# krea-ai/realtime-video

Hardware: AMD Instinct MI355X
Metric: frames/sec at 832x480, 4-step 14B T2V (per-step DiT latency in config) (higher is better)
Workload: dtype bf16

## Files before the change

__graft_entry__.py:

```python
import os
import sys

ROOT = os.path.dirname(os.path.abspath(__file__))
if ROOT not in sys.path:
    sys.path.insert(0, ROOT)


def build() -> None:
    from realtime_video_amd import _lib
    _lib.build(verbose=False)
    import realtime_video_amd.attention
    import realtime_video_amd.causal_model
    import realtime_video_amd.pipeline
    import realtime_video_amd.session
    import realtime_video_amd.taehv
    import realtime_video_amd.vae_decoder
    lib = _lib.load()
    missing = [s for s in _lib.declared_symbols() if not hasattr(lib, s)]
    if missing:
        raise RuntimeError(f"librtv_hip.so lacks symbols declared in include/rtv_hip.h: {missing}")
    import re
    import subprocess
    def audit(script, *argv, **env):
        r = subprocess.run([os.path.join(ROOT, "scripts", "micro", script), *argv], capture_output=True, text=True,
                           env=dict(os.environ, **env))
        return r.stdout + ("\n[stderr]\n" + r.stderr if r.stderr.strip() else "") + (f"\n[exit {r.returncode}]" if r.returncode else "")

    out = audit("w4_audit.sh", "600", W4_AUDIT_DIR=os.path.join(ROOT, "realtime_video_amd", "csrc", "build", "w4_audit"))
    ok = all(re.search(pat, out) for pat in (r"accumulation register outside asm: 0\b", r"v_accvgpr outside asm: 0\b", r"\bscratch 0\b",
                                              r"vgpr_spill_count: 0\b", r"private_segment_fixed_size: 0\b"))
    if not ok:
        raise RuntimeError("attn_w4 audit failed (scripts/micro/w4_audit.sh):\n" + out)
    out = audit("g5_audit.sh", G5_AUDIT_DIR=os.path.join(ROOT, "realtime_video_amd", "csrc", "build", "g5_audit"))
    if len(re.findall(r"AUDIT gemm5 F16=\d: vgpr_spills 0 private_segment 0 scratch_ops 0 mfma 120 compiler_acc_refs_before_last_accumulator_read 0 ", out)) != 2:
        raise RuntimeError("gemm5 audit failed (scripts/micro/g5_audit.sh):\n" + out)
    out = audit("h4_audit.sh", H4_AUDIT_DIR=os.path.join(ROOT, "realtime_video_amd", "csrc", "build", "h4_audit"))
    if len(re.findall(r"AUDIT _ZN3rtv1[78]conv_halo4p?_kernel\S*: arch_vgprs \d+ vgpr_spills 0 sgpr_spills \d+ private_segment 0 scratch_ops 0 "
                      r"mfma 216 compiler_acc_refs 0 \(a0-a7: 0\)", out)) != 2:
        raise RuntimeError("conv_halo4 audit failed (scripts/micro/h4_audit.sh):\n" + out)
    print(f"build ok: {_lib.LIB_PATH} ({len(_lib.declared_symbols())} C-ABI symbols; attn_w4 / gemm5 / conv_halo4 register audits clean)")


def smoke() -> None:
    import torch
    from oracle import vae_oracle as vo
    from oracle import wan_oracle as wo
    from realtime_video_amd.causal_model import CausalWanModel
    from realtime_video_amd.vae_decoder import VAEDecoderWrapper
    from realtime_video_amd.wan_wrapper import WanDiffusionWrapper

    assert torch.cuda.is_available(), "smoke() needs a GPU"
    dev = "cuda:0"
    torch.cuda.set_device(0)
    cfg = dict(dim=256, ffn_dim=512, num_heads=2, num_layers=1, freq_dim=256, text_len=512, eps=1e-6)
    w = wo.make_weights(cfg, seed=1, text_dim=64)
    g = torch.Generator().manual_seed(2)
    lat = torch.randn(1, 3, 16, 60, 104, generator=g).to(torch.bfloat16)
    ctx = torch.randn(32, 64, generator=g).to(torch.bfloat16)
    t = torch.tensor([[500.0, 500.0, 500.0]])
    kvc = wo.initialize_kv_cache(1, 1, 9360, 2, 128, torch.bfloat16)
    cac = wo.initialize_crossattn_cache(1, 1, 2, 128, torch.bfloat16)
    ref, _ = wo.wrapper_forward(w, cfg, wo.FlowMatchScheduler(), lat, [ctx], t, kvc, cac, 0)

    model = CausalWanModel(dim=256, ffn_dim=512, num_heads=2, num_layers=1, text_dim=64, device=dev)
    model.load_state_dict(w)
    wr = WanDiffusionWrapper(model, timestep_shift=5.0)
    kv = [{"k": torch.zeros(1, 9360, 2, 128, dtype=torch.bfloat16, device=dev),
           "v": torch.zeros(1, 9360, 2, 128, dtype=torch.bfloat16, device=dev), "global_end_index": 0, "local_end_index": 0}]
    ca = [{"k": torch.zeros(1, 512, 2, 128, dtype=torch.bfloat16, device=dev),
           "v": torch.zeros(1, 512, 2, 128, dtype=torch.bfloat16, device=dev), "is_init": False}]
    flow, _ = wr(lat.to(dev), {"prompt_embeds": [ctx.to(dev)]}, t.to(dev), kv, ca, current_start=0)
    torch.cuda.synchronize()
    err = float((flow.cpu().double() - ref.double()).norm() / ref.double().norm())
# ... 20 lines not shown
```

realtime_video_amd/_lib.py:

```python
import ctypes
import os
import re
import subprocess

_HERE = os.path.dirname(os.path.abspath(__file__))
LIB_PATH = os.environ.get("RTV_LIB_PATH") or os.path.join(_HERE, "librtv_hip.so")
CSRC = os.path.join(_HERE, "csrc")

_INCLUDE = os.path.join(os.path.dirname(_HERE), "include")
HEADERS = ("rtv_hip.h", "rtv_hip_lab.h")

_lib = None

_SCALARS = {"int": ctypes.c_int, "int64_t": ctypes.c_int64, "float": ctypes.c_float, "double": ctypes.c_double,
            "size_t": ctypes.c_size_t}
_RETURNS = {"int": ctypes.c_int, "size_t": ctypes.c_size_t, "const char*": ctypes.c_char_p}
_STARS = r"(\*(?:\s*const\s*\*)?)?"


def _field_type(base, stars, structs):
    value = _SCALARS.get(base) or structs.get(base)
    if not stars:
        return value
    if base == "void":
# ... 57 lines not shown

STRUCTS, PROTOTYPES = {}, {}
for _name in HEADERS:
    PROTOTYPES.update(parse_header(_read(_name), STRUCTS))
IO_HEADER = "rtv_hip_io.h"
IO_STRUCTS = dict(STRUCTS)
IO_PROTOTYPES = parse_header(_read(IO_HEADER), IO_STRUCTS)
IO_STRUCTS = {k: v for k, v in IO_STRUCTS.items() if k not in STRUCTS}
JPEG_HEADER = "rtv_hip_jpeg.h"
JPEG_STRUCTS = dict(STRUCTS)
JPEG_PROTOTYPES = parse_header(_read(JPEG_HEADER), JPEG_STRUCTS)
JPEG_STRUCTS = {k: v for k, v in JPEG_STRUCTS.items() if k not in STRUCTS}
JPEGDEC_HEADER = "rtv_hip_jpeg_decode.h"
JPEGDEC_STRUCTS = dict(STRUCTS)
JPEGDEC_PROTOTYPES = parse_header(_read(JPEGDEC_HEADER), JPEGDEC_STRUCTS)
JPEGDEC_STRUCTS = {k: v for k, v in JPEGDEC_STRUCTS.items() if k not in STRUCTS}
LORA_HEADER = "rtv_hip_lora.h"
LORA_STRUCTS = dict(STRUCTS)
LORA_PROTOTYPES = parse_header(_read(LORA_HEADER), LORA_STRUCTS)
LORA_STRUCTS = {k: v for k, v in LORA_STRUCTS.items() if k not in STRUCTS}
CROSS_FOLD_HEADER = "rtv_hip_cross_fold.h"
CROSS_FOLD_STRUCTS = dict(STRUCTS)
CROSS_FOLD_PROTOTYPES = parse_header(_read(CROSS_FOLD_HEADER), CROSS_FOLD_STRUCTS)
FP8_ROWS_HEADER = "rtv_hip_fp8_rows.h"
FP8_ROWS_PROTOTYPES = parse_header(_read(FP8_ROWS_HEADER), dict(STRUCTS))
ATTN_FP8_HEADER = "rtv_hip_attn_fp8.h"
ATTN_FP8_STRUCTS = dict(STRUCTS)
ATTN_FP8_PROTOTYPES = parse_header(_read(ATTN_FP8_HEADER), ATTN_FP8_STRUCTS)
ATTN_FP8_STRUCTS = {k: v for k, v in ATTN_FP8_STRUCTS.items() if k not in STRUCTS}
MXFP4_HEADER = "rtv_hip_mxfp4.h"
MXFP4_PROTOTYPES = parse_header(_read(MXFP4_HEADER), dict(STRUCTS))
MXFP6_HEADER = "rtv_hip_mxfp6.h"
MXFP6_PROTOTYPES = parse_header(_read(MXFP6_HEADER), dict(STRUCTS))
LORA_MAX_ADAPTERS, LORA_MAX_RANK = (int(re.search(rf"^#define\s+RTV_LORA_MAX_{n}\s+(\d+)", _read(LORA_HEADER), flags=re.M).group(1))
                                    for n in ("ADAPTERS", "RANK"))
FRAMES_MAX = int(re.search(r"^#define\s+RTV_FRAMES_MAX\s+(\d+)", _read(IO_HEADER), flags=re.M).group(1))
ABI_VERSION = int(re.search(r"^#define\s+RTV_ABI_VERSION\s+(\d+)", _read(HEADERS[0]), flags=re.M).group(1))


def build(verbose=False):
    jobs = os.environ.get("MAX_JOBS") or str(min(16, len(os.sched_getaffinity(0)) if hasattr(os, "sched_getaffinity") else os.cpu_count() or 4))
    cmd = ["make", "-C", CSRC, "-j", jobs]
    res = subprocess.run(cmd, capture_output=True, text=True)
    if verbose or res.returncode != 0:
        print(res.stdout[-4000:])
        print(res.stderr[-4000:])
    if res.returncode != 0:
        raise RuntimeError("building librtv_hip.so failed")
    return LIB_PATH


def declared_symbols(lab=True):
    out = set()
    for name in HEADERS if lab else HEADERS[:1]:
        text = re.sub(r"/\*.*?\*/", "", _read(name), flags=re.S)
        out.update(re.findall(r"\b(rtv_[a-z0-9_]+)\s*\(", text))
    return sorted(out)


def load():
    global _lib
    if _lib is not None:
        return _lib
    if not os.path.exists(LIB_PATH):
        raise RuntimeError(
            f"{LIB_PATH} is missing: run `python -c 'import __graft_entry__ as g; g.build()'` "
            "(or `make -C realtime_video_amd/csrc`). There is no CPU fallback for the HIP path.")
    lib = ctypes.CDLL(LIB_PATH)
    for name, (restype, argtypes) in list(PROTOTYPES.items()) + list(IO_PROTOTYPES.items()) + list(JPEG_PROTOTYPES.items()) + list(JPEGDEC_PROTOTYPES.items()) + list(LORA_PROTOTYPES.items()) + list(CROSS_FOLD_PROTOTYPES.items()) + list(FP8_ROWS_PROTOTYPES.items()) + list(ATTN_FP8_PROTOTYPES.items()) + list(MXFP4_PROTOTYPES.items()) + list(MXFP6_PROTOTYPES.items()):
        fn = getattr(lib, name, None)
        if fn is None:
            if os.environ.get("RTV_LIB_PATH"):
                continue
            raise RuntimeError(f"librtv_hip.so does not export {name}")
        fn.restype, fn.argtypes = restype, argtypes
    have = lib.rtv_version()
    if have != ABI_VERSION:
        raise RuntimeError(f"{LIB_PATH} reports ABI revision {have}, include/rtv_hip.h declares RTV_ABI_VERSION {ABI_VERSION}: "
                           "rebuild the library (`make -C realtime_video_amd/csrc`)")
    _lib = lib
    return lib


def check(status, what):
    if status != 0:
        msg = load().rtv_last_error().decode("utf-8", "replace")
        raise RuntimeError(f"{what} failed (status {status}): {msg}")


def call(name, *args):
    check(getattr(load(), name)(*args), name)
```

realtime_video_amd/csrc/dit_forward.hip:

```cpp
#include <atomic>
#include <string>

#include "../../include/rtv_hip_attn_fp8.h"
#include "../../include/rtv_hip_mxfp4.h"
#include "../../include/rtv_hip_mxfp6.h"
#include "rtv_common.h"
#include "rtv_internal.h"

namespace rtv {

__global__ void silu_kernel(const bf16_t* __restrict__ x, bf16_t* __restrict__ out, int64_t n) {
  for (int64_t i = (int64_t)blockIdx.x * blockDim.x + threadIdx.x; i < n; i += (int64_t)gridDim.x * blockDim.x)
    out[i] = f32_to_bf16(silu(bf16_to_f32(x[i])));
}

constexpr int FOLD_ROWS = 64, FOLD_LD = 130;
__global__ __launch_bounds__(256) void cross_fold_weight_kernel(const bf16_t* __restrict__ w, int64_t ldw, const bf16_t* __restrict__ v,
                                                               int64_t ldv, bf16_t* __restrict__ vo, int64_t ldvo, int H, int rows, int kh,
                                                               int k_fold) {
  __shared__ __attribute__((aligned(16))) bf16_t sW[FOLD_ROWS * FOLD_LD];
  __shared__ __attribute__((aligned(16))) bf16_t sV[128 * FOLD_LD];
  const int tid = threadIdx.x, lane = tid & 63, wave = tid >> 6;
  const int n0 = blockIdx.x * FOLD_ROWS, h = blockIdx.y;
  for (int id = tid; id < FOLD_ROWS * 64; id += 256) {
// ... 290 lines not shown
  const int pk = cfg->in_dim * 4;
  RTV_TRY(rtv_patchify(st->x, b.prow, cfg->in_dim, F, c.gh, c.gw, stream));
  RTV_TRY(linear(c, -1, b.prow + (size_t)c.r0 * pk, pk, w->patch_w, w->patch_b, b.x, c.rc, d, 0, nullptr, 0, 0, 0, nullptr, tc, stream));
  RTV_TRY(rtv_sinusoidal_embedding(st->t, b.sinus, F, cfg->freq_dim, stream));
  RTV_TRY(linear(c, S_TIME0, b.sinus, cfg->freq_dim, w->time0_w, w->time0_b, b.te1, F, d, RTV_ACT_SILU, nullptr, 0, 0, 0, nullptr, tc, stream));
  RTV_TRY(linear(c, S_TIME2, b.te1, d, w->time2_w, w->time2_b, b.e, F, d, 0, nullptr, 0, 0, 0, nullptr, tc, stream));
  RTV_TRY(rtv_silu(b.e, b.se, (int64_t)F * d, stream));
  RTV_TRY(linear(c, S_TPROJ, b.se, d, w->tproj_w, w->tproj_b, b.e0, F, 6 * d, 0, nullptr, 0, 0, 0, nullptr, tc, stream));
  RTV_TRY(rtv_modulation_table(w->modulation, b.e0, b.emod, L, F, 6, 6, d, stream));
  RTV_TRY(rtv_modulation_table(w->head_modulation, b.e, b.ehead, 1, F, 2, 1, d, stream));
  if (st->compute_cross_kv) {
    if (!st->context) return set_error(-1, "dit: context required to initialise the cross-attention cache");
    const int T = cfg->text_len;
    RTV_TRY(linear(c, S_TEXT0, st->context, cfg->text_dim, w->text0_w, w->text0_b, b.ctx1, T, d, RTV_ACT_GELU_TANH, nullptr, 0, 0, 0, nullptr, tc, stream));
    RTV_TRY(linear(c, S_TEXT2, b.ctx1, d, w->text2_w, w->text2_b, b.ctx, T, d, 0, nullptr, 0, 0, 0, nullptr, tc, stream));
    for (int l = 0; l < L; ++l) {
      const rtv_dit_layer_weights& lw = w->layers[l];
      RTV_TRY(linear(c, S_LAYER0 + S_PER_LAYER * l + S_CK, b.ctx, d, lw.ck_w, lw.ck_b, b.ktmp, T, d, 0, nullptr, 0, 0, 0, nullptr, tc, stream));
      RTV_TRY(rtv_rmsnorm(b.ktmp, d, st->ca_k[l], d, T, d, cfg->eps, lw.cnorm_k_w, stream));
      RTV_TRY(linear(c, S_LAYER0 + S_PER_LAYER * l + S_CV, b.ctx, d, lw.cv_w, lw.cv_b, st->ca_v[l], T, d, 0, nullptr, 0, 0, 0, nullptr, tc, stream));
      if (c.fold_k)
        RTV_TRY(rtv_cross_fold_weight(lw.co_w, d, st->ca_v[l], d, st->ca_v[c.L + l], st->ca_vo_ld, c.H, st->text_rows + 1, c.fold_kh, c.fold_k,
                                      stream));
    }
  }
  return 0;
}

static int hp_check(Ctx& c, int world);
static int quantize_written_rows(Ctx& c, int l);

static std::atomic<void*> g_capture_q{nullptr}, g_capture_o{nullptr};
static std::atomic<int> g_direct_v{1};
static int dit_layer_proj(Ctx& c, int l, int parts, int world, void* q_send, void* kv_send) {
  const rtv_dit_layer_weights& lw = c.w->layers[l];
  const rtv_dit_step* st = c.st;
  DitBuffers& b = c.b;
  const int d = c.d;
  if (!(parts & (RTV_PROJ_LN | RTV_PROJ_Q | RTV_PROJ_KV))) return set_error(-1, "dit: empty projection phase");
  const uint16_t* em = b.emod + (size_t)l * c.F * 6 * d;
  if (parts & RTV_PROJ_LN) {
    const void* ln_out;
    RTV_TRY(ln_input(c, em + 0 * d, em + 1 * d, 6 * d, nullptr, nullptr, &ln_out));
  }
  const bool q = parts & RTV_PROJ_Q, kv = parts & RTV_PROJ_KV;
  if (!q && !kv) return 0;
  const int n0 = q ? 0 : d, nn = (q ? d : 0) + (kv ? 2 * d : 0);
  bool v_in_place = false;
  {
    void* v_dst = nullptr;
    if (kv && !kv_send && g_direct_v.load(std::memory_order_relaxed) && st->kv_v[l] && !(st->kv_row_stride & 7)) {
      int r0 = st->cache_row0 + c.r0;
      const int S = st->ring_lo, R = st->ring_size;
      bool one_range = true;
      if (R > 0 && r0 + c.rc > S) {
        if (r0 < S) one_range = false;
        else {
          r0 = S + (r0 - S + st->ring_shift) % R;
          one_range = r0 + c.rc <= S + R;
        }
      }
      uint16_t* dst = (uint16_t*)st->kv_v[l] + (size_t)r0 * st->kv_row_stride;
      if (one_range && !((uintptr_t)dst & 15)) v_dst = dst;
    }
    {
      const int rp = (q ? 1 : 0) | (kv ? 2 : 0) | (v_dst ? 4 : 0);
      if (q_send || kv_send) {
        RTV_TRY(hp_check(c, world));
        const int gc = d / world;
        if ((q && !q_send) || (kv && !kv_send)) return set_error(-1, "dit: exchange buffers required");
        RTV_TRY(qk_norm_rope_check(2 * gc, 0, c.rc, d, c.H, c.F, c.gh, c.gw, st->start_frame, c.r0, gc, (int64_t)c.rc * gc,
                                   (int64_t)c.rc * 2 * gc, 0, 0, 0, rp));
      } else {
        RTV_TRY(qk_norm_rope_check(st->kv_row_stride, st->cache_row0, c.rc, d, c.H, c.F, c.gh, c.gw, st->start_frame, c.r0, 0, 0, 0,
                                   st->ring_lo, st->ring_size, st->ring_shift, rp));
      }
    }
    const int sidx = S_LAYER0 + S_PER_LAYER * l + S_QKV;
    const void* a = c.cfg->use_fp8 >= FP8_ROWS ? nullptr : b.xn;
    RTV_TRY(quantize_input(c, sidx, a, c.rc, d, c.stream));
    auto proj = [&](int w_row0, int N, void* out, int ldc) {
      return project(c, sidx, a, d, lw.qkv_w, w_row0, lw.qkv_b, out, ldc, c.rc, N, 0, nullptr, 0, 0, 0, nullptr, c.tc, c.stream);
    };
    if (v_dst) {
      if (2 * d > n0) RTV_TRY(proj(n0, 2 * d - n0, b.qkv + n0, 3 * d));
      RTV_TRY(proj(2 * d, d, v_dst, (int)st->kv_row_stride));
      v_in_place = true;
    } else {
      RTV_TRY(proj(n0, nn, b.qkv + n0, 3 * d));
    }
  }
  const int rope_parts = (q ? 1 : 0) | (kv ? 2 : 0) | (v_in_place ? 4 : 0);
  if (q_send || kv_send) {
    RTV_TRY(hp_check(c, world));
    const int gc = d / world;
    if ((q && !q_send) || (kv && !kv_send)) return set_error(-1, "dit: exchange buffers required");
    return qk_norm_rope_launch(b.qkv, q_send, kv_send, kv_send ? (void*)((uint16_t*)kv_send + gc) : nullptr, 2 * gc, 0, c.rc, d, c.H,
                               c.cfg->eps, lw.norm_q_w, lw.norm_k_w, c.w->rope_cs, c.F, c.gh, c.gw, st->start_frame, c.r0, gc,
                               (int64_t)c.rc * gc, (int64_t)c.rc * 2 * gc, 0, 0, 0, rope_parts, c.stream);
  }
  RTV_TRY(qk_norm_rope_launch(b.qkv, b.q, st->kv_k[l], st->kv_v[l], st->kv_row_stride, st->cache_row0, c.rc, d, c.H, c.cfg->eps,
                              lw.norm_q_w, lw.norm_k_w, c.w->rope_cs, c.F, c.gh, c.gw, st->start_frame, c.r0, 0, 0, 0, st->ring_lo,
                              st->ring_size, st->ring_shift, rope_parts, c.stream));
  if (kv && c.fp8) return quantize_written_rows(c, l);
  return 0;
}

static int quantize_written_rows(Ctx& c, int l) {
  const rtv_dit_step* st = c.st;
  const rtv_attn_fp8_shadow* sh = c.fp8;
  if (!sh->k8[l] || !sh->v8t[l]) return set_error(-1, "dit: fp8 attention: a layer has no shadow");
  int a = st->cache_row0 + c.r0, n = c.rc;
  const int S = st->ring_lo, R = st->ring_size;
  int seg[3][2], ns = 0;
  if (R <= 0) {
    seg[ns][0] = a, seg[ns++][1] = n;
  } else {
    if (a < S) {
      const int m = n < S - a ? n : S - a;
      seg[ns][0] = a, seg[ns++][1] = m;
      a += m, n -= m;
    }
    if (n > 0) {
      const int p0 = S + (a - S + st->ring_shift) % R;
      const int first = n < S + R - p0 ? n : S + R - p0;
      seg[ns][0] = p0, seg[ns++][1] = first;
      if (n - first > R) return set_error(-1, "dit: fp8 attention: a call writes more rows than the ring holds");
      if (n > first) seg[ns][0] = S, seg[ns++][1] = n - first;
    }
  }
  void* amax = sh->amax ? sh->amax[l] : nullptr;
  for (int i = 0; i < ns; ++i)
    RTV_TRY(rtv_attn_quantize_kv(st->kv_k[l], st->kv_v[l], st->kv_row_stride, seg[i][0], seg[i][1], c.H, sh->k8[l], sh->v8t[l],
                                 sh->cache_rows, sh->k_scale, sh->v_scale, amax, c.stream));
  return 0;
}
// ... 236 lines not shown
  RTV_TRY(dit_begin(c));
  for (int l = 0; l < c.L; ++l) {
    if (st->kv_only && l == c.L - 1)
      return dit_layer_proj(c, l, RTV_PROJ_LN | RTV_PROJ_KV, 0, nullptr, nullptr);
    RTV_TRY(dit_layer_qkv(c, l));
    RTV_TRY(dit_layer_rest(c, l));
  }
  RTV_TRY(dit_head(c, c.b.hrow));
  return rtv_unpatchify(c.b.hrow, st->out, cfg->out_dim, c.F, c.gh, c.gw, stream);
}

extern "C" int rtv_dit_forward(const rtv_dit_config* cfg, const rtv_dit_weights* w, const rtv_dit_step* st,
                               void* workspace, size_t workspace_bytes, rtv_stream_t stream) {
  return dit_forward(cfg, w, st, nullptr, workspace, workspace_bytes, stream);
}

extern "C" int rtv_dit_forward_attn_fp8(const rtv_dit_config* cfg, const rtv_dit_weights* w, const rtv_dit_step* st,
                                        const rtv_attn_fp8_shadow* shadow, void* workspace, size_t workspace_bytes,
                                        rtv_stream_t stream) {
  if (!shadow) return set_error(-1, "dit: fp8 attention needs its shadow (rtv_attn_fp8_shadow)");
  return dit_forward(cfg, w, st, shadow, workspace, workspace_bytes, stream);
}

extern "C" int rtv_dit_lab_capture_self_attn(void* q_copy, void* o_copy) {
  g_capture_q = q_copy;
  g_capture_o = o_copy;
  return 0;
}

extern "C" int rtv_dit_set_direct_v(int on) {
  g_direct_v = on ? 1 : 0;
  return 0;
}
```

realtime_video_amd/csrc/elementwise.hip:

```cpp
#include "ln_row.h"
#include "rtv_common.h"
#include "rtv_internal.h"

namespace rtv {

static std::atomic<int> g_rope_wave{-1};
constexpr int ROPE_WAVE_MIN_ROWS = 2048;

__global__ __launch_bounds__(EW_THREADS) void layernorm_modulate_kernel(
    const bf16_t* __restrict__ x, bf16_t* __restrict__ out, int d, float eps,
    const bf16_t* __restrict__ shift, const bf16_t* __restrict__ scale, int frame_stride,
    int rows_per_frame, int row_offset, const bf16_t* __restrict__ weight, const bf16_t* __restrict__ bias) {
  __shared__ float red[8];
  bf16_t* orow = out + (size_t)blockIdx.x * d;
  layernorm_row(x, d, eps, shift, scale, frame_stride, rows_per_frame, row_offset, weight, bias, red,
                [&](int, int c, const float* o) { *(u32x4*)(orow + c * 8) = pack_bf16x8(o); });
}

__global__ __launch_bounds__(EW_THREADS) void rmsnorm_kernel(const bf16_t* __restrict__ x, int ldx,
                                                             bf16_t* __restrict__ out, int ldo, int d,
                                                             float eps,
                                                             const bf16_t* __restrict__ weight) {
  __shared__ float red[8];
  const int row = blockIdx.x;
// ... 35 lines not shown
}

constexpr int ROWS_PER_WG = 4;

struct RopeArgs {
  const bf16_t* qkv;
  bf16_t* q_out;
  bf16_t* k_cache;
  bf16_t* v_cache;
  int64_t cache_row_stride;
  int cache_row0;
  int M, d, hd;
  float eps;
  const bf16_t* wq;
  const bf16_t* wk;
  const float2* rope_cs;
  int gh, gw, start_frame, row_offset;
  int group_cols;
  int64_t q_group_stride, kv_group_stride;
  int ring_lo, ring_size, ring_shift;
  int parts;
};

__device__ __forceinline__ void rope8(float* x, const float2* w) {
#pragma unroll
  for (int t = 0; t < 4; ++t) {
    const float a = x[2 * t], b = x[2 * t + 1];
    x[2 * t] = a * w[t].x - b * w[t].y;
    x[2 * t + 1] = a * w[t].y + b * w[t].x;
  }
}

template <int CPL, bool LANE_CS>
__global__ __launch_bounds__(EW_THREADS) __attribute__((amdgpu_waves_per_eu(CPL <= 10 ? 5 : 3, 8))) void qk_norm_rope_cache_kernel(RopeArgs a) {
  const int lane = threadIdx.x & 63;
  const bool do_q = a.parts & 1, do_kv = a.parts & 2;
  const int nroles = do_kv ? 2 : 1;
  const int wid = __builtin_amdgcn_readfirstlane(blockIdx.x * ROWS_PER_WG + (threadIdx.x >> 6));
  const int row = wid / nroles, role = wid - row * nroles;
  if (row >= a.M) return;
  const int d = a.d;
  const int nchunks = d >> 3;
  const bf16_t* qr = a.qkv + (size_t)row * 3 * d;
  const bf16_t* vr = qr + 2 * d;
  const bool norm = role == 1 || do_q;
  const bf16_t* xr = role == 1 ? qr + d : qr;
  const bf16_t* wx = role == 1 ? a.wk : a.wq;

  const int half = a.hd >> 1;
  const int c1 = half / 3, c0 = half - 2 * c1;
  const int per_frame = a.gh * a.gw;
  const int grow = a.row_offset + row;
  const int f = grow / per_frame;
  const int rem = grow - f * per_frame;
  const int pos_h = rem / a.gw, pos_w = rem - pos_h * a.gw;
  const int pos_f = a.start_frame + f;
  auto load_cs = [&](int col, float2* w) {
    const int pj0 = (col % a.hd) >> 1;
#pragma unroll
    for (int t = 0; t < 4; ++t) {
      const int pj = pj0 + t;
      const int pos = pj < c0 ? pos_f : (pj < c0 + c1 ? pos_h : pos_w);
      w[t] = a.rope_cs[pos * half + pj];
    }
  };
  float2 cs[4];
  if (LANE_CS && norm) load_cs(lane * 8, cs);

  const int gc = a.group_cols;
  size_t kv_row = gc ? (size_t)row : (size_t)(a.cache_row0 + grow);
  if (!gc && a.ring_size > 0 && (int)kv_row >= a.ring_lo)
    kv_row = (size_t)(a.ring_lo + ((int)kv_row - a.ring_lo + a.ring_shift) % a.ring_size);
  bf16_t* xo = role == 1 ? a.k_cache + kv_row * a.cache_row_stride : a.q_out + (size_t)row * (gc ? gc : d);
  const int64_t x_group_stride = role == 1 ? a.kv_group_stride : a.q_group_stride;
  bf16_t* vo = a.v_cache + kv_row * a.cache_row_stride;

  u32x4 raw[CPL];
  if (norm) {
#pragma unroll
    for (int i = 0; i < CPL; ++i) {
      const int c = lane + i * 64;
      if (c < nchunks) raw[i] = *(const u32x4*)(xr + c * 8);
    }
  }
  if (do_kv && !(a.parts & 4)) {
    constexpr int VH = (CPL + 1) / 2;
    const int i0 = role * VH;
    u32x4 vraw[VH];
#pragma unroll
    for (int i = 0; i < VH; ++i) {
      const int c = lane + (i0 + i) * 64;
      if (i0 + i < CPL && c < nchunks) vraw[i] = *(const u32x4*)(vr + c * 8);
    }
#pragma unroll
    for (int i = 0; i < VH; ++i) {
      const int c = lane + (i0 + i) * 64;
      if (i0 + i < CPL && c < nchunks) {
        const int g = gc ? (c * 8) / gc : 0;
        *(u32x4*)(vo + g * a.kv_group_stride + (c * 8 - g * gc)) = vraw[i];
      }
    }
  }
  if (!norm) return;
  float acc4[4] = {0.f, 0.f, 0.f, 0.f};
#pragma unroll
  for (int i = 0; i < CPL; ++i) {
    if (lane + i * 64 < nchunks) {
      float t[8];
      unpack_bf16x8(raw[i], t);
#pragma unroll
      for (int j = 0; j < 8; ++j) acc4[i & 3] = __builtin_fmaf(t[j], t[j], acc4[i & 3]);
    }
  }
  const float sx = ((acc4[0] + acc4[1]) + acc4[2]) + acc4[3];
  const float rx = rsqrtf(wave_sum(sx) / (float)d + a.eps);
  asm volatile("" ::: "memory");
#pragma unroll
  for (int i = 0; i < CPL; ++i) launder(raw[i]);
#pragma unroll
  for (int i = 0; i < CPL; ++i) {
    const int c = lane + i * 64;
    if (c < nchunks) {
      const int g = gc ? (c * 8) / gc : 0;
      const int col = c * 8 - g * gc;
      float2 wc[4];
      if (!LANE_CS) load_cs(c * 8, wc);
      float w8[8], x[8];
      unpack_bf16x8(*(const u32x4*)(wx + c * 8), w8);
      unpack_bf16x8(raw[i], x);
#pragma unroll
      for (int j = 0; j < 8; ++j) x[j] = round_bf16(round_bf16(x[j] * rx) * w8[j]);
      rope8(x, LANE_CS ? cs : wc);
      *(u32x4*)(xo + g * x_group_stride + col) = pack_bf16x8(x);
    }
  }
}

__device__ __forceinline__ void block_sum2(float& a, float& b, float* red ) {
  const int l = threadIdx.x & 63;
  red[threadIdx.x] = a;
  red[256 + threadIdx.x] = b;
  __syncthreads();
  a = wave_sum(((red[l] + red[64 + l]) + red[128 + l]) + red[192 + l]);
  b = wave_sum(((red[256 + l] + red[320 + l]) + red[384 + l]) + red[448 + l]);
}

__device__ __forceinline__ void rope8_cols(float* x, int col, int hd, int c0, int c1, int pos_f, int pos_h,
                                      int pos_w, const float2* __restrict__ cs) {
  const int half = hd >> 1;
  const int pj0 = (col % hd) >> 1;
#pragma unroll
  for (int t = 0; t < 4; ++t) {
    int pj = pj0 + t;
    int pos = pj < c0 ? pos_f : (pj < c0 + c1 ? pos_h : pos_w);
// ... 144 lines not shown
    int xh = (int)(t % Hh);
    t /= Hh;
    int f = (int)(t % F);
    int c = (int)(t / F);
    int h = xh >> 1, q = xh & 1, w = xw >> 1, r = xw & 1;
    size_t m = ((size_t)f * gh + h) * gw + w;
    x[i] = rows[m * (C * 4) + (q * 2 + r) * C + c];
  }
}

}

namespace rtv {
int qk_norm_rope_check(int64_t cache_row_stride, int cache_row0, int M, int d, int num_heads, int F, int gh, int gw, int start_frame,
                       int row_offset, int group_cols, int64_t q_group_stride, int64_t kv_group_stride, int ring_lo, int ring_size,
                       int ring_shift, int parts) {
  if (M <= 0) return 0;
  if (parts < 1 || parts > 7 || parts == 4 || parts == 5) return set_error(-1, "qk_norm_rope_cache: parts must be 1 (q), 2 (k, v) or 3 (+ 4: V in place)");
  if (ring_size < 0 || ring_lo < 0 || ring_shift < 0 || (ring_size > 0 && ring_shift >= ring_size))
    return set_error(-1, "qk_norm_rope_cache: bad ring (need ring_lo >= 0, 0 <= ring_shift < ring_size)");
  if (ring_size > 0 && cache_row0 + row_offset + M > ring_lo + ring_size)
    return set_error(-1, "qk_norm_rope_cache: rows beyond the end of the ring");
  if (num_heads <= 0 || d % num_heads) return set_error(-1, "qk_norm_rope_cache: d % num_heads != 0");
  const int hd = d / num_heads;
  if (d % 8 || d > EW_THREADS * 8 * EW_MAXC || hd % 8 || cache_row_stride % 8)
    return set_error(-1, "qk_norm_rope_cache: alignment (d, head_dim, cache stride multiples of 8; d <= 8192)");
  if (row_offset < 0 || row_offset + M > F * gh * gw) return set_error(-1, "qk_norm_rope_cache: rows outside the F*gh*gw token grid");
  if (start_frame < 0 || start_frame + F > 1024 || gh > 1024 || gw > 1024)
    return set_error(-1, "qk_norm_rope_cache: position exceeds the 1024-entry RoPE table");
  if (cache_row0 < 0) return set_error(-1, "qk_norm_rope_cache: negative cache row");
  if (group_cols && (group_cols % hd || d % group_cols || q_group_stride % 8 || kv_group_stride % 8))
    return set_error(-1, "qk_norm_rope_cache: head groups must be whole heads dividing d");
  return 0;
}

int qk_norm_rope_launch(const void* qkv, void* q_out, void* k_cache, void* v_cache, int64_t cache_row_stride,
                        int cache_row0, int M, int d, int num_heads, float eps, const void* wq, const void* wk,
                        const void* rope_cs, int F, int gh, int gw, int start_frame, int row_offset, int group_cols,
                        int64_t q_group_stride, int64_t kv_group_stride, int ring_lo, int ring_size, int ring_shift,
                        int parts, rtv_stream_t stream) {
  if (M <= 0) return 0;
  if (qk_norm_rope_check(cache_row_stride, cache_row0, M, d, num_heads, F, gh, gw, start_frame, row_offset, group_cols, q_group_stride,
                         kv_group_stride, ring_lo, ring_size, ring_shift, parts))
    return -1;
  const int hd = d / num_heads;
  RopeArgs a;
  a.qkv = (const bf16_t*)qkv;
  a.q_out = (bf16_t*)q_out;
  a.k_cache = (bf16_t*)k_cache;
  a.v_cache = (bf16_t*)v_cache;
  a.cache_row_stride = cache_row_stride;
  a.cache_row0 = cache_row0;
  a.M = M;
  a.d = d;
  a.hd = hd;
  a.eps = eps;
  a.wq = (const bf16_t*)wq;
  a.wk = (const bf16_t*)wk;
  a.rope_cs = (const float2*)rope_cs;
  a.gh = gh;
  a.gw = gw;
  a.start_frame = start_frame;
  a.row_offset = row_offset;
  a.group_cols = group_cols;
  a.q_group_stride = q_group_stride;
  a.kv_group_stride = kv_group_stride;
  a.ring_lo = ring_lo;
  a.ring_size = ring_size;
  a.ring_shift = ring_shift;
  a.parts = parts;
  ProfScope prof(PROF_ROPE, (hipStream_t)stream, ((parts & 1 ? 2.0 : 0.0) + (parts & 2 ? (parts & 4 ? 2.0 : 4.0) : 0.0)) * M * d * 2);
  const int g_sel = g_rope_wave.load(std::memory_order_relaxed);
  if (g_sel == 0 || (g_sel < 0 && M < ROPE_WAVE_MIN_ROWS)) {
    hipLaunchKernelGGL(qk_norm_rope_cache_block_kernel, dim3(M), dim3(EW_THREADS), 0, (hipStream_t)stream, a);
    return check_launch("qk_norm_rope_cache");
  }
  const int waves = M * ((parts & 2) ? 2 : 1);
  const dim3 grid((waves + ROWS_PER_WG - 1) / ROWS_PER_WG);
#define RTV_ROPE_CALL(CPL)                                                                                                  \
  if (512 % hd == 0) hipLaunchKernelGGL((qk_norm_rope_cache_kernel<CPL, true>), grid, dim3(EW_THREADS), 0, (hipStream_t)stream, a); \
  else hipLaunchKernelGGL((qk_norm_rope_cache_kernel<CPL, false>), grid, dim3(EW_THREADS), 0, (hipStream_t)stream, a)
  RTV_ROW_DISPATCH(d, RTV_ROPE_CALL);
#undef RTV_ROPE_CALL
  return check_launch("qk_norm_rope_cache");
}

__global__ void regroup_heads_kernel(const u32x4* __restrict__ in, u32x4* __restrict__ out, int rows, int G, int gc8) {
  const size_t total = (size_t)rows * G * gc8;
  for (size_t i = (size_t)blockIdx.x * blockDim.x + threadIdx.x; i < total; i += (size_t)gridDim.x * blockDim.x) {
    const int c = (int)(i % gc8);
    const size_t t = i / gc8;
    const int g = (int)(t % G);
    const size_t r = t / G;
    out[i] = in[((size_t)g * rows + r) * gc8 + c];
  }
}

__global__ void pixels_to_rgb8_kernel(const float* __restrict__ px, uint8_t* __restrict__ out, int T, size_t hw) {
  const size_t quads = hw >> 2;
  const size_t total = (size_t)T * quads;
  for (size_t i = (size_t)blockIdx.x * blockDim.x + threadIdx.x; i < total; i += (size_t)gridDim.x * blockDim.x) {
    const size_t t = i / quads, q = i - t * quads;
    const float* base = px + t * 3 * hw + q * 4;
    float4 c[3];
#pragma unroll
    for (int ch = 0; ch < 3; ++ch) c[ch] = *(const float4*)(base + ch * hw);
// ... 68 lines not shown

int rtv_pixels_to_rgb8(const void* pixels, void* rgb8, int T, int H, int W, rtv_stream_t stream) {
  if (T <= 0 || H <= 0 || W <= 0) return 0;
  if (!pixels || !rgb8) return set_error(-1, "pixels_to_rgb8: null argument");
  const size_t hw = (size_t)H * W;
  if (hw % 4 || ((uintptr_t)pixels & 15) || ((uintptr_t)rgb8 & 3))
    return set_error(-1, "pixels_to_rgb8: H*W must be a multiple of 4, pixels 16-byte and rgb8 4-byte aligned");
  const size_t total = (size_t)T * (hw / 4);
  int blocks = (int)((total + 255) / 256);
  if (blocks > 8192) blocks = 8192;
  ProfScope prof(PROF_MISC, (hipStream_t)stream, (double)T * hw * 15.0);
  hipLaunchKernelGGL(pixels_to_rgb8_kernel, dim3(blocks), dim3(256), 0, (hipStream_t)stream, (const float*)pixels,
                     (uint8_t*)rgb8, T, hw);
  return check_launch("pixels_to_rgb8");
}

int rtv_qk_norm_rope_cache(const void* qkv, void* q_out, void* k_cache, void* v_cache,
                           int64_t cache_row_stride, int cache_row0, int M, int d, int num_heads, float eps,
                           const void* wq, const void* wk, const void* rope_cs, int F, int gh, int gw,
                           int start_frame, int row_offset, rtv_stream_t stream) {
  return rtv::qk_norm_rope_launch(qkv, q_out, k_cache, v_cache, cache_row_stride, cache_row0, M, d, num_heads, eps, wq, wk,
                                  rope_cs, F, gh, gw, start_frame, row_offset, 0, 0, 0, 0, 0, 0, 3, stream);
}

int rtv_qk_norm_rope_cache_ring(const void* qkv, void* q_out, void* k_cache, void* v_cache,
                                int64_t cache_row_stride, int cache_row0, int M, int d, int num_heads, float eps,
                                const void* wq, const void* wk, const void* rope_cs, int F, int gh, int gw,
                                int start_frame, int row_offset, int ring_lo, int ring_size, int ring_shift,
                                rtv_stream_t stream) {
  return rtv::qk_norm_rope_launch(qkv, q_out, k_cache, v_cache, cache_row_stride, cache_row0, M, d, num_heads, eps, wq, wk,
                                  rope_cs, F, gh, gw, start_frame, row_offset, 0, 0, 0, ring_lo, ring_size, ring_shift, 3, stream);
}

int rtv_modulation_table(const void* modulation, const void* e0, void* emod, int L, int F, int J, int J0,
                         int d, rtv_stream_t stream) {
  if (J0 != J && J0 != 1) return set_error(-1, "modulation_table: J0 must be J or 1");
  size_t total = (size_t)L * F * J * d;
  if (total == 0) return 0;
  int blocks = (int)((total + 255) / 256);
  if (blocks > 4096) blocks = 4096;
  ProfScope prof(PROF_MISC, (hipStream_t)stream, (double)total * 6);
  hipLaunchKernelGGL(modulation_table_kernel, dim3(blocks), dim3(256), 0, (hipStream_t)stream,
                     (const bf16_t*)modulation, (const bf16_t*)e0, (bf16_t*)emod, L, F, J, J0, d);
  return check_launch("modulation_table");
}

int rtv_sinusoidal_embedding(const void* t, void* out, int F, int dim, rtv_stream_t stream) {
  if (dim % 2) return set_error(-1, "sinusoidal_embedding: dim must be even");
  int n = F * (dim / 2);
  if (n <= 0) return 0;
  hipLaunchKernelGGL(sinusoidal_kernel, dim3((n + 127) / 128), dim3(128), 0, (hipStream_t)stream,
                     (const float*)t, (bf16_t*)out, F, dim);
  return check_launch("sinusoidal_embedding");
}

int rtv_patchify(const void* x, void* rows, int C, int F, int gh, int gw, rtv_stream_t stream) {
  size_t total = (size_t)F * gh * gw * C * 4;
  if (total == 0) return 0;
  int blocks = (int)((total + 255) / 256);
  if (blocks > 4096) blocks = 4096;
  hipLaunchKernelGGL(patchify_kernel, dim3(blocks), dim3(256), 0, (hipStream_t)stream, (const bf16_t*)x,
                     (bf16_t*)rows, C, F, gh, gw);
  return check_launch("patchify");
}

int rtv_unpatchify(const void* rows, void* x, int C, int F, int gh, int gw, rtv_stream_t stream) {
// ... 11 lines not shown
```

realtime_video_amd/csrc/rtv_internal.h:

```cpp
#pragma once
#include <hip/hip_runtime.h>

#include <atomic>

#include "../../include/rtv_hip.h"
#include "../../include/rtv_hip_cross_fold.h"
#include "../../include/rtv_hip_fp8_rows.h"
#include "../../include/rtv_hip_lab.h"

namespace rtv {

int set_error(int code, const char* msg);
int check_launch(const char* what);

struct LdsAttr {
  std::atomic<uint64_t> done{0};
};
int ensure_dynamic_lds(const void* kernel, int bytes, LdsAttr* state, const char* what);

int device_num_cus();

enum ProfClass { PROF_GEMM = 0, PROF_ATTN, PROF_LN, PROF_ROPE, PROF_CONV, PROF_MISC, PROF_NCLASS };

struct ProfScope {
  ProfScope(int cls, hipStream_t stream, double work);
  ~ProfScope();
  int slot;
  hipStream_t stream;
};

enum DispatchKernel {
  DK_GEMM_128x128 = 0, DK_GEMM_OTHER_CFG, DK_GEMM8_256x256, DK_GEMM8M_128x256, DK_GEMM5_160x256, DK_GEMM_FP8_256x256,
  DK_ATTN_W4, DK_ATTN_FOUR_PHASE, DK_ATTN_LOCKSTEP_256ROW, DK_ATTN_LOCKSTEP_128ROW, DK_ATTN_SPLIT_COMBINE,
  DK_CONV_HALO4P, DK_CONV_HALO4, DK_CONV_HALO, DK_CONV_IGEMM, DK_ATTN_PROBS, DK_GEMM_MXFP4_256x256, DK_GEMM_MXFP6_256x256, DK_COUNT
};
void note_kernel(int id);

struct GemmParams;
int launch_gemm(const GemmParams& p, int dtype, int tile_cfg, hipStream_t stream);
int launch_gemm8(const GemmParams& p, bool f16, bool split_k, hipStream_t stream);
int launch_gemm4(const GemmParams& p, bool f16, hipStream_t stream, int lab = 0);
int launch_gemm8m(const GemmParams& p, bool f16, bool split_k, hipStream_t stream);
int launch_gemm5(const GemmParams& p, bool f16, bool split_k, hipStream_t stream);
int launch_quantize_fp8(const uint16_t* x, int64_t ld, int M, int d, uint8_t* q, int64_t ldq, float* scale_out,
                        unsigned* amax_scratch, hipStream_t stream);
int launch_gemm_fp8(GemmParams p, const uint8_t* A, int lda, const uint8_t* W, int ldw, const float* a_scale, float w_scale,
                    hipStream_t stream);
int launch_gemm_fp8_rows(GemmParams p, const uint8_t* A, int lda, const uint8_t* W, int ldw, const float* a_scales,
                         const float* w_scales, hipStream_t stream);

int qk_norm_rope_check(int64_t cache_row_stride, int cache_row0, int M, int d, int num_heads, int F, int gh, int gw, int start_frame,
                       int row_offset, int group_cols, int64_t q_group_stride, int64_t kv_group_stride, int ring_lo, int ring_size,
                       int ring_shift, int parts);
int qk_norm_rope_launch(const void* qkv, void* q_out, void* k_cache, void* v_cache, int64_t cache_row_stride,
                        int cache_row0, int M, int d, int num_heads, float eps, const void* wq, const void* wk,
                        const void* rope_cs, int F, int gh, int gw, int start_frame, int row_offset, int group_cols,
                        int64_t q_group_stride, int64_t kv_group_stride, int ring_lo, int ring_size, int ring_shift,
                        int parts , rtv_stream_t stream);
int regroup_heads(const void* in, void* out, int rows, int G, int group_cols, rtv_stream_t stream);

int conv3_last_tap(const void* frame, const void* w3, const void* bias, const void* gamma, const void* residual, int res_ld, void* out,
                   int out_ld, int H, int W, int Cin, int Cout, int flags, const void* zeros, hipStream_t stream);

}
```

realtime_video_amd/csrc/runtime.hip:

```cpp
#include <mutex>
#include <string>
#include <vector>

#include "gemm_core.h"
#include "rtv_internal.h"

namespace rtv {

static thread_local std::string g_err;

int set_error(int code, const char* msg) {
  g_err = msg ? msg : "unknown error";
  if (code > 0) {
    g_err += ": ";
    g_err += hipGetErrorString((hipError_t)code);
  }
  return code == 0 ? -1 : code;
}

int ensure_dynamic_lds(const void* kernel, int bytes, LdsAttr* state, const char* what) {
  int dev = 0;
  if (hipGetDevice(&dev) != hipSuccess || dev < 0 || dev >= 64) return set_error(-1, "cannot query the current device");
  const uint64_t bit = 1ull << dev;
  if (state->done.load(std::memory_order_acquire) & bit) return 0;
// ... 49 lines not shown
static std::vector<hipEvent_t> g_event_pool;

static hipEvent_t get_event() {
  if (!g_event_pool.empty()) {
    hipEvent_t e = g_event_pool.back();
    g_event_pool.pop_back();
    return e;
  }
  hipEvent_t e;
  hipEventCreate(&e);
  return e;
}

ProfScope::ProfScope(int cls, hipStream_t s, double work) : slot(-1), stream(s) {
  if (!((g_prof_mask >> cls) & 1u)) return;
  std::lock_guard<std::mutex> lk(g_prof_mu);
  g_prof_seen_work[cls] += work;
  if (g_prof_seen[cls]++ % g_prof_stride[cls]) return;
  ProfRec r;
  r.cls = cls;
  r.work = work;
  r.start = get_event();
  r.stop = get_event();
  hipEventRecord(r.start, s);
  g_prof.push_back(r);
  slot = (int)g_prof.size() - 1;
}
ProfScope::~ProfScope() {
  if (slot < 0) return;
  std::lock_guard<std::mutex> lk(g_prof_mu);
  hipEventRecord(g_prof[slot].stop, stream);
}

}

using namespace rtv;

extern "C" {

int rtv_version(void) { return RTV_ABI_VERSION; }

const char* rtv_last_error(void) { return g_err.c_str(); }

int rtv_lab_build(void) {
#ifdef RTV_LAB
  return 1;
#else
  return 0;
#endif
}

int rtv_dispatch_counts(int64_t* counts, int n) {
  for (int i = 0; counts && i < n && i < DK_COUNT; ++i) counts[i] = g_dispatch[i].load(std::memory_order_relaxed);
  return DK_COUNT;
}

const char* rtv_dispatch_name(int id) { return id >= 0 && id < DK_COUNT ? g_dispatch_names[id] : ""; }

int rtv_dispatch_reset(void) {
  for (auto& c : g_dispatch) c.store(0, std::memory_order_relaxed);
  return 0;
}

int rtv_prof_enable(int class_mask) {
  g_prof_mask = (unsigned)class_mask;
  return 0;
}

int rtv_prof_reset(void) {
  std::lock_guard<std::mutex> lk(g_prof_mu);
  for (auto& r : g_prof) {
    g_event_pool.push_back(r.start);
    g_event_pool.push_back(r.stop);
// ... 91 lines not shown
```

Baseline: 19.26.

## Overlap QK-norm/RoPE cache kernel with V projection on a side stream

Adds an optional side-stream fork/join so the Q/K norm+RoPE+cache kernel runs concurrently with the V-projection GEMM when not capturing a graph. Also moves the raw row load after the V-copy branch with clamped indices, raises the min waves-per-EU hint for small CPL, and adds a register audit for the rope kernels. The overlap is disabled by default (RTV_ROPE_OVERLAP=0), so only the kernel tweaks apply by default. The overlap path risks contention between concurrent kernels and adds event overhead.

```diff
diff --git a/__graft_entry__.py b/__graft_entry__.py
--- a/__graft_entry__.py
+++ b/__graft_entry__.py
@@ -38,7 +38,11 @@
     if len(re.findall(r"AUDIT _ZN3rtv1[78]conv_halo4p?_kernel\S*: arch_vgprs \d+ vgpr_spills 0 sgpr_spills \d+ private_segment 0 scratch_ops 0 "
                       r"mfma 216 compiler_acc_refs 0 \(a0-a7: 0\)", out)) != 2:
         raise RuntimeError("conv_halo4 audit failed (scripts/micro/h4_audit.sh):\n" + out)
-    print(f"build ok: {_lib.LIB_PATH} ({len(_lib.declared_symbols())} C-ABI symbols; attn_w4 / gemm5 / conv_halo4 register audits clean)")
+    out = audit("rope_audit.sh", ROPE_AUDIT_DIR=os.path.join(ROOT, "realtime_video_amd", "csrc", "build", "rope_audit"))
+    rope = re.findall(r"AUDIT rope CPL=(?:2|4|10) \S+: vgprs \d+ allocated (\d+) vgpr_spills 0 private_segment 0 lds 0 scratch_ops 0 barriers 0\b", out)
+    if len(rope) != 6 or any(int(v) > 80 for v in rope):
+        raise RuntimeError("RoPE / cache kernel audit failed (scripts/micro/rope_audit.sh):\n" + out)
+    print(f"build ok: {_lib.LIB_PATH} ({len(_lib.declared_symbols())} C-ABI symbols; attn_w4 / gemm5 / conv_halo4 / rope register audits clean)")
 
 
 def smoke() -> None:
diff --git a/include/rtv_hip_rope_overlap.h b/include/rtv_hip_rope_overlap.h
--- /dev/null
+++ b/include/rtv_hip_rope_overlap.h
@@ -0,0 +1,18 @@
+#ifndef RTV_HIP_ROPE_OVERLAP_H
+#define RTV_HIP_ROPE_OVERLAP_H
+#ifdef __cplusplus
+extern "C" {
+#endif
+
+int rtv_dit_set_rope_overlap(int mode);
+int rtv_side_streams_release(void);
+
+int rtv_qk_norm_rope_cache_parts(const void* qkv, void* q_out, void* k_cache, void* v_cache, int64_t cache_row_stride, int cache_row0,
+                                 int M, int d, int num_heads, float eps, const void* wq, const void* wk, const void* rope_cs, int F,
+                                 int gh, int gw, int start_frame, int row_offset, int ring_lo, int ring_size, int ring_shift,
+                                 int parts, rtv_stream_t stream);
+
+#ifdef __cplusplus
+}
+#endif
+#endif
diff --git a/realtime_video_amd/_lib.py b/realtime_video_amd/_lib.py
--- a/realtime_video_amd/_lib.py
+++ b/realtime_video_amd/_lib.py
@@ -113,6 +113,8 @@
 MXFP4_PROTOTYPES = parse_header(_read(MXFP4_HEADER), dict(STRUCTS))
 MXFP6_HEADER = "rtv_hip_mxfp6.h"
 MXFP6_PROTOTYPES = parse_header(_read(MXFP6_HEADER), dict(STRUCTS))
+ROPE_OVERLAP_HEADER = "rtv_hip_rope_overlap.h"
+ROPE_OVERLAP_PROTOTYPES = parse_header(_read(ROPE_OVERLAP_HEADER), dict(STRUCTS))
 LORA_MAX_ADAPTERS, LORA_MAX_RANK = (int(re.search(rf"^#define\s+RTV_LORA_MAX_{n}\s+(\d+)", _read(LORA_HEADER), flags=re.M).group(1))
                                     for n in ("ADAPTERS", "RANK"))
 FRAMES_MAX = int(re.search(r"^#define\s+RTV_FRAMES_MAX\s+(\d+)", _read(IO_HEADER), flags=re.M).group(1))
@@ -148,7 +150,7 @@
             f"{LIB_PATH} is missing: run `python -c 'import __graft_entry__ as g; g.build()'` "
             "(or `make -C realtime_video_amd/csrc`). There is no CPU fallback for the HIP path.")
     lib = ctypes.CDLL(LIB_PATH)
-    for name, (restype, argtypes) in list(PROTOTYPES.items()) + list(IO_PROTOTYPES.items()) + list(JPEG_PROTOTYPES.items()) + list(JPEGDEC_PROTOTYPES.items()) + list(LORA_PROTOTYPES.items()) + list(CROSS_FOLD_PROTOTYPES.items()) + list(FP8_ROWS_PROTOTYPES.items()) + list(ATTN_FP8_PROTOTYPES.items()) + list(MXFP4_PROTOTYPES.items()) + list(MXFP6_PROTOTYPES.items()):
+    for name, (restype, argtypes) in list(PROTOTYPES.items()) + list(IO_PROTOTYPES.items()) + list(JPEG_PROTOTYPES.items()) + list(JPEGDEC_PROTOTYPES.items()) + list(LORA_PROTOTYPES.items()) + list(CROSS_FOLD_PROTOTYPES.items()) + list(FP8_ROWS_PROTOTYPES.items()) + list(ATTN_FP8_PROTOTYPES.items()) + list(MXFP4_PROTOTYPES.items()) + list(MXFP6_PROTOTYPES.items()) + list(ROPE_OVERLAP_PROTOTYPES.items()):
         fn = getattr(lib, name, None)
         if fn is None:
             if os.environ.get("RTV_LIB_PATH"):
diff --git a/realtime_video_amd/csrc/dit_forward.hip b/realtime_video_amd/csrc/dit_forward.hip
--- a/realtime_video_amd/csrc/dit_forward.hip
+++ b/realtime_video_amd/csrc/dit_forward.hip
@@ -346,6 +346,12 @@
 
 static std::atomic<void*> g_capture_q{nullptr}, g_capture_o{nullptr};
 static std::atomic<int> g_direct_v{1};
+constexpr int ROPE_OVERLAP_DEFAULT = 0;
+static int rope_overlap_from_env() {
+  const char* e = getenv("RTV_ROPE_OVERLAP");
+  return e && e[0] >= '0' && e[0] <= '2' && !e[1] ? e[0] - '0' : ROPE_OVERLAP_DEFAULT;
+}
+static std::atomic<int> g_rope_overlap{rope_overlap_from_env()};
 static int dit_layer_proj(Ctx& c, int l, int parts, int world, void* q_send, void* kv_send) {
   const rtv_dit_layer_weights& lw = c.w->layers[l];
   const rtv_dit_step* st = c.st;
@@ -361,6 +367,11 @@
   if (!q && !kv) return 0;
   const int n0 = q ? 0 : d, nn = (q ? d : 0) + (kv ? 2 * d : 0);
   bool v_in_place = false;
+  auto rope_local = [&](int rope_parts, rtv_stream_t s) {
+    return qk_norm_rope_launch(b.qkv, b.q, st->kv_k[l], st->kv_v[l], st->kv_row_stride, st->cache_row0, c.rc, d, c.H, c.cfg->eps,
+                               lw.norm_q_w, lw.norm_k_w, c.w->rope_cs, c.F, c.gh, c.gw, st->start_frame, c.r0, 0, 0, 0, st->ring_lo,
+                               st->ring_size, st->ring_shift, rope_parts, s);
+  };
   {
     void* v_dst = nullptr;
     if (kv && !kv_send && g_direct_v.load(std::memory_order_relaxed) && st->kv_v[l] && !(st->kv_row_stride & 7)) {
@@ -398,6 +409,27 @@
     };
     if (v_dst) {
       if (2 * d > n0) RTV_TRY(proj(n0, 2 * d - n0, b.qkv + n0, 3 * d));
+      const int ov = g_rope_overlap.load(std::memory_order_relaxed);
+      bool fork = ov && q && kv && (parts & RTV_PROJ_LN) && !q_send && c.rc == c.M && (ov == 2 || qk_norm_rope_wave_form(c.rc));
+      if (fork) {
+        hipStreamCaptureStatus cap = hipStreamCaptureStatusNone;
+        if (hipStreamIsCapturing((hipStream_t)c.stream, &cap) != hipSuccess) {
+          (void)hipGetLastError();
+          fork = false;
+        } else {
+          fork = cap == hipStreamCaptureStatusNone;
+        }
+      }
+      if (fork) {
+        hipStream_t side;
+        RTV_TRY(side_fork((hipStream_t)c.stream, &side));
+        int r = rope_local(3 | 4, (rtv_stream_t)side);
+        if (!r) r = proj(2 * d, d, v_dst, (int)st->kv_row_stride);
+        const int rj = side_join((hipStream_t)c.stream);
+        if (r || rj) return r ? r : rj;
+        if (c.fp8) return quantize_written_rows(c, l);
+        return 0;
+      }
       RTV_TRY(proj(2 * d, d, v_dst, (int)st->kv_row_stride));
       v_in_place = true;
     } else {
@@ -413,9 +445,7 @@
                                c.cfg->eps, lw.norm_q_w, lw.norm_k_w, c.w->rope_cs, c.F, c.gh, c.gw, st->start_frame, c.r0, gc,
                                (int64_t)c.rc * gc, (int64_t)c.rc * 2 * gc, 0, 0, 0, rope_parts, c.stream);
   }
-  RTV_TRY(qk_norm_rope_launch(b.qkv, b.q, st->kv_k[l], st->kv_v[l], st->kv_row_stride, st->cache_row0, c.rc, d, c.H, c.cfg->eps,
-                              lw.norm_q_w, lw.norm_k_w, c.w->rope_cs, c.F, c.gh, c.gw, st->start_frame, c.r0, 0, 0, 0, st->ring_lo,
-                              st->ring_size, st->ring_shift, rope_parts, c.stream));
+  RTV_TRY(rope_local(rope_parts, c.stream));
   if (kv && c.fp8) return quantize_written_rows(c, l);
   return 0;
 }
@@ -718,3 +748,9 @@
   g_direct_v = on ? 1 : 0;
   return 0;
 }
+
+extern "C" int rtv_dit_set_rope_overlap(int mode) {
+  if (mode < 0 || mode > 2) return set_error(-1, "dit_set_rope_overlap: 0 (off), 1 (on) or 2 (on at every row count)");
+  g_rope_overlap = mode;
+  return 0;
+}
diff --git a/realtime_video_amd/csrc/elementwise.hip b/realtime_video_amd/csrc/elementwise.hip
--- a/realtime_video_amd/csrc/elementwise.hip
+++ b/realtime_video_amd/csrc/elementwise.hip
@@ -91,7 +91,7 @@
 }
 
 template <int CPL, bool LANE_CS>
-__global__ __launch_bounds__(EW_THREADS) __attribute__((amdgpu_waves_per_eu(CPL <= 10 ? 5 : 3, 8))) void qk_norm_rope_cache_kernel(RopeArgs a) {
+__global__ __launch_bounds__(EW_THREADS) __attribute__((amdgpu_waves_per_eu(CPL <= 10 ? 6 : 3, 8))) void qk_norm_rope_cache_kernel(RopeArgs a) {
   const int lane = threadIdx.x & 63;
   const bool do_q = a.parts & 1, do_kv = a.parts & 2;
   const int nroles = do_kv ? 2 : 1;
@@ -134,14 +134,6 @@
   const int64_t x_group_stride = role == 1 ? a.kv_group_stride : a.q_group_stride;
   bf16_t* vo = a.v_cache + kv_row * a.cache_row_stride;
 
-  u32x4 raw[CPL];
-  if (norm) {
-#pragma unroll
-    for (int i = 0; i < CPL; ++i) {
-      const int c = lane + i * 64;
-      if (c < nchunks) raw[i] = *(const u32x4*)(xr + c * 8);
-    }
-  }
   if (do_kv && !(a.parts & 4)) {
     constexpr int VH = (CPL + 1) / 2;
     const int i0 = role * VH;
@@ -161,6 +153,12 @@
     }
   }
   if (!norm) return;
+  u32x4 raw[CPL];
+#pragma unroll
+  for (int i = 0; i < CPL; ++i) {
+    const int c = lane + i * 64;
+    raw[i] = *(const u32x4*)(xr + (c < nchunks ? c : nchunks - 1) * 8);
+  }
   float acc4[4] = {0.f, 0.f, 0.f, 0.f};
 #pragma unroll
   for (int i = 0; i < CPL; ++i) {
@@ -176,9 +174,11 @@
   asm volatile("" ::: "memory");
 #pragma unroll
   for (int i = 0; i < CPL; ++i) launder(raw[i]);
+  int lane2 = lane;
+  asm volatile("" : "+v"(lane2));
 #pragma unroll
   for (int i = 0; i < CPL; ++i) {
-    const int c = lane + i * 64;
+    const int c = lane2 + i * 64;
     if (c < nchunks) {
       const int g = gc ? (c * 8) / gc : 0;
       const int col = c * 8 - g * gc;
@@ -389,6 +389,11 @@
   if (group_cols && (group_cols % hd || d % group_cols || q_group_stride % 8 || kv_group_stride % 8))
     return set_error(-1, "qk_norm_rope_cache: head groups must be whole heads dividing d");
   return 0;
+}
+
+bool qk_norm_rope_wave_form(int M) {
+  const int sel = g_rope_wave.load(std::memory_order_relaxed);
+  return sel > 0 || (sel < 0 && M >= ROPE_WAVE_MIN_ROWS);
 }
 
 int qk_norm_rope_launch(const void* qkv, void* q_out, void* k_cache, void* v_cache, int64_t cache_row_stride,
@@ -427,8 +432,7 @@
   a.ring_shift = ring_shift;
   a.parts = parts;
   ProfScope prof(PROF_ROPE, (hipStream_t)stream, ((parts & 1 ? 2.0 : 0.0) + (parts & 2 ? (parts & 4 ? 2.0 : 4.0) : 0.0)) * M * d * 2);
-  const int g_sel = g_rope_wave.load(std::memory_order_relaxed);
-  if (g_sel == 0 || (g_sel < 0 && M < ROPE_WAVE_MIN_ROWS)) {
+  if (!qk_norm_rope_wave_form(M)) {
     hipLaunchKernelGGL(qk_norm_rope_cache_block_kernel, dim3(M), dim3(EW_THREADS), 0, (hipStream_t)stream, a);
     return check_launch("qk_norm_rope_cache");
   }
@@ -563,6 +567,15 @@
                                   rope_cs, F, gh, gw, start_frame, row_offset, 0, 0, 0, ring_lo, ring_size, ring_shift, 3, stream);
 }
 
+int rtv_qk_norm_rope_cache_parts(const void* qkv, void* q_out, void* k_cache, void* v_cache,
+                                 int64_t cache_row_stride, int cache_row0, int M, int d, int num_heads, float eps,
+                                 const void* wq, const void* wk, const void* rope_cs, int F, int gh, int gw,
+                                 int start_frame, int row_offset, int ring_lo, int ring_size, int ring_shift, int parts,
+                                 rtv_stream_t stream) {
+  return rtv::qk_norm_rope_launch(qkv, q_out, k_cache, v_cache, cache_row_stride, cache_row0, M, d, num_heads, eps, wq, wk,
+                                  rope_cs, F, gh, gw, start_frame, row_offset, 0, 0, 0, ring_lo, ring_size, ring_shift, parts, stream);
+}
+
 int rtv_modulation_table(const void* modulation, const void* e0, void* emod, int L, int F, int J, int J0,
                          int d, rtv_stream_t stream) {
   if (J0 != J && J0 != 1) return set_error(-1, "modulation_table: J0 must be J or 1");
diff --git a/realtime_video_amd/csrc/rtv_internal.h b/realtime_video_amd/csrc/rtv_internal.h
--- a/realtime_video_amd/csrc/rtv_internal.h
+++ b/realtime_video_amd/csrc/rtv_internal.h
@@ -7,6 +7,7 @@
 #include "../../include/rtv_hip_cross_fold.h"
 #include "../../include/rtv_hip_fp8_rows.h"
 #include "../../include/rtv_hip_lab.h"
+#include "../../include/rtv_hip_rope_overlap.h"
 
 namespace rtv {
 
@@ -28,6 +29,9 @@
   int slot;
   hipStream_t stream;
 };
+
+int side_fork(hipStream_t main, hipStream_t* side);
+int side_join(hipStream_t main);
 
 enum DispatchKernel {
   DK_GEMM_128x128 = 0, DK_GEMM_OTHER_CFG, DK_GEMM8_256x256, DK_GEMM8M_128x256, DK_GEMM5_160x256, DK_GEMM_FP8_256x256,
@@ -57,6 +61,7 @@
                         const void* rope_cs, int F, int gh, int gw, int start_frame, int row_offset, int group_cols,
                         int64_t q_group_stride, int64_t kv_group_stride, int ring_lo, int ring_size, int ring_shift,
                         int parts , rtv_stream_t stream);
+bool qk_norm_rope_wave_form(int M);
 int regroup_heads(const void* in, void* out, int rows, int G, int group_cols, rtv_stream_t stream);
 
 int conv3_last_tap(const void* frame, const void* w3, const void* bias, const void* gamma, const void* residual, int res_ld, void* out,
diff --git a/realtime_video_amd/csrc/runtime.hip b/realtime_video_amd/csrc/runtime.hip
--- a/realtime_video_amd/csrc/runtime.hip
+++ b/realtime_video_amd/csrc/runtime.hip
@@ -105,6 +105,63 @@
   hipEventRecord(g_prof[slot].stop, stream);
 }
 
+constexpr int SIDE_EVENTS = 8;
+struct SideLane {
+  hipStream_t stream = nullptr;
+  hipEvent_t ev[SIDE_EVENTS] = {};
+  int next = 0;
+};
+static std::mutex g_side_mu;
+static SideLane g_side[64];
+
+static int side_lane(SideLane** out) {
+  int dev = 0;
+  if (hipGetDevice(&dev) != hipSuccess || dev < 0 || dev >= 64) return set_error(-1, "side stream: cannot query the current device");
+  SideLane& s = g_side[dev];
+  if (!s.stream) {
+    hipStream_t st = nullptr;
+    hipError_t e = hipStreamCreateWithFlags(&st, hipStreamNonBlocking);
+    if (e != hipSuccess) return set_error((int)e, "side stream: hipStreamCreateWithFlags");
+    for (int i = 0; i < SIDE_EVENTS; ++i) {
+      e = hipEventCreateWithFlags(&s.ev[i], hipEventDisableTiming);
+      if (e != hipSuccess) {
+        for (int j = 0; j < i; ++j) (void)hipEventDestroy(s.ev[j]);
+        (void)hipStreamDestroy(st);
+        return set_error((int)e, "side stream: hipEventCreateWithFlags");
+      }
+    }
+    s.stream = st;
+    s.next = 0;
+  }
+  *out = &s;
+  return 0;
+}
+
+static int side_order(SideLane& s, hipStream_t from, hipStream_t to) {
+  hipEvent_t ev = s.ev[s.next];
+  s.next = (s.next + 1) % SIDE_EVENTS;
+  hipError_t e = hipEventRecord(ev, from);
+  if (e != hipSuccess) return set_error((int)e, "side stream: hipEventRecord");
+  e = hipStreamWaitEvent(to, ev, 0);
+  if (e != hipSuccess) return set_error((int)e, "side stream: hipStreamWaitEvent");
+  return 0;
+}
+
+int side_fork(hipStream_t main, hipStream_t* side) {
+  std::lock_guard<std::mutex> lk(g_side_mu);
+  SideLane* s;
+  if (int r = side_lane(&s)) return r;
+  *side = s->stream;
+  return side_order(*s, main, s->stream);
+}
+
+int side_join(hipStream_t main) {
+  std::lock_guard<std::mutex> lk(g_side_mu);
+  SideLane* s;
+  if (int r = side_lane(&s)) return r;
+  return side_order(*s, s->stream, main);
+}
+
 }
 
 using namespace rtv;
@@ -112,6 +169,19 @@
 extern "C" {
 
 int rtv_version(void) { return RTV_ABI_VERSION; }
+
+int rtv_side_streams_release(void) {
+  std::lock_guard<std::mutex> lk(g_side_mu);
+  int rc = 0;
+  for (SideLane& s : g_side) {
+    if (!s.stream) continue;
+    for (hipEvent_t& e : s.ev) (void)hipEventDestroy(e), e = nullptr;
+    const hipError_t e = hipStreamDestroy(s.stream);
+    if (e != hipSuccess) rc = set_error((int)e, "side_streams_release: hipStreamDestroy");
+    s.stream = nullptr;
+  }
+  return rc;
+}
 
 const char* rtv_last_error(void) { return g_err.c_str(); }
 
```

Result: no change. 19.29, median of 3 (+0.2%).
